# Yubo-Shankui/Bind-Your-Avatar-Implementation

Hardware: AMD Instinct MI355X
Metric: denoise-steps/sec (higher is better)
Workload: dtype bf16; 1 GPU; BASELINE.json configs[1]: full transformer.forward, 49x480x720 (13x30x45 latent tokens + 226 text), 2 characters (2 ID + 2 audio), batch 1, random-init 8.6B-param architecture; layers=42, batch=1, launch=eager, parallelism=single GPU

## Files before the change

bind_your_avatar_implementation_amd/csrc/attn_w4.hip:

```cpp
#ifndef BYA_ATTN_W4_BODY
#include "attn_common.h"
#include "gemm_persistent.h"
#include <stdlib.h>
#include "options.h"

namespace {

template <char C> struct IntTagC { static constexpr char value = C; };

constexpr int QB = 4;
constexpr int ROWS_PER_WG = 4 * QB * 32;
constexpr int RB = 128, TILE_BYTES = KV_TILE * RB, STAGE_BYTES = 2 * TILE_BYTES, NST = 3;

struct SkItem { int bh, qt, tb, nt, nt_all, role, local, slot; };

constexpr int SK_SLOT_FLOATS = 4 * QB * 2 * 16 * 64 + 4 * QB * 64;
constexpr int SK_FLAG_BYTES = 4096;

#define BYA_ATTN_W4_BODY
template <bool SK>
__global__ __launch_bounds__(256, 1) void attn_joint_w4_kernel(AttnArgs p) {
    constexpr int MXF = -1;
    const AttnMxOut* const mx = nullptr;
#include __FILE__
// ... 234 lines not shown
            MASKPAD(sacc[1][1], 32);
            { float t1_0; float t1_1; float t1_2; float t1_3; float t1_4; float t1_5; float t1_6; float t1_7; float t1_8; float t1_9; float t1_10; float t1_11; float t1_12; float t1_13; float t1_14; float t1_15; uint32_t w2_0; uint32_t w2_1; uint32_t w2_2; uint32_t w2_3; uint32_t w3_0; uint32_t w3_1; uint32_t w3_2; uint32_t w3_3; asm volatile("v_mfma_f32_32x32x16_bf16 %0, %28, %29, 0\n\tv_exp_f32 %1, %30\n\tv_exp_f32 %2, %31\n\tv_mfma_f32_32x32x16_bf16 %0, %32, %33, %0\n\tv_exp_f32 %3, %34\n\tv_add_f32 %5, %5, %1\n\tv_exp_f32 %4, %35\n\tv_add_f32 %6, %6, %2\n\tv_cvt_pk_bf16_f32 %7, %1, %2\n\tv_mfma_f32_32x32x16_bf16 %0, %36, %37, %0\n\tv_exp_f32 %8, %38\n\tv_add_f32 %5, %5, %3\n\tv_exp_f32 %9, %39\n\tv_add_f32 %6, %6, %4\n\tv_cvt_pk_bf16_f32 %10, %3, %4\n\tv_mfma_f32_32x32x16_bf16 %0, %40, %41, %0\n\tv_exp_f32 %11, %42\n\tv_add_f32 %5, %5, %8\n\tv_exp_f32 %12, %43\n\tv_add_f32 %6, %6, %9\n\tv_cvt_pk_bf16_f32 %13, %8, %9\n\tv_mfma_f32_32x32x16_bf16 %14, %44, %29, 0\n\tv_exp_f32 %15, %45\n\tv_add_f32 %5, %5, %11\n\tv_exp_f32 %16, %46\n\tv_add_f32 %6, %6, %12\n\tv_cvt_pk_bf16_f32 %17, %11, %12\n\tv_mfma_f32_32x32x16_bf16 %14, %47, %33, %14\n\tv_exp_f32 %18, %48\n\tv_add_f32 %5, %5, %15\n\tv_exp_f32 %19, %49\n\tv_add_f32 %6, %6, %16\n\tv_cvt_pk_bf16_f32 %20, %15, %16\n\tv_mfma_f32_32x32x16_bf16 %14, %50, %37, %14\n\tv_exp_f32 %21, %51\n\tv_add_f32 %5, %5, %18\n\tv_exp_f32 %22, %52\n\tv_add_f32 %6, %6, %19\n\tv_cvt_pk_bf16_f32 %23, %18, %19\n\tv_mfma_f32_32x32x16_bf16 %14, %53, %41, %14\n\tv_exp_f32 %24, %54\n\tv_add_f32 %5, %5, %21\n\tv_exp_f32 %25, %55\n\tv_add_f32 %6, %6, %22\n\tv_cvt_pk_bf16_f32 %26, %21, %22\n\tv_add_f32 %5, %5, %24\n\tv_add_f32 %6, %6, %25\n\tv_cvt_pk_bf16_f32 %27, %24, %25" : "=&v"(sacc[0][0]), "=&v"(t1_0), "=&v"(t1_1), "=&v"(t1_2), "=&v"(t1_3), "+v"(psum[1][0]), "+v"(psum[1][1]), "=&v"(w2_0), "=&v"(t1_4), "=&v"(t1_5), "=&v"(w2_1), "=&v"(t1_6), "=&v"(t1_7), "=&v"(w2_2), "=&v"(sacc[0][1]), "=&v"(t1_8), "=&v"(t1_9), "=&v"(w2_3), "=&v"(t1_10), "=&v"(t1_11), "=&v"(w3_0), "=&v"(t1_12), "=&v"(t1_13), "=&v"(w3_1), "=&v"(t1_14), "=&v"(t1_15), "=&v"(w3_2), "=&v"(w3_3) : "v"(kf[0][0]), "a"(qf[2][0]), "v"(sacc[1][1][0]), "v"(sacc[1][1][1]), "v"(kf[0][1]), "a"(qf[2][1]), "v"(sacc[1][1][2]), "v"(sacc[1][1][3]), "v"(kf[0][2]), "a"(qf[2][2]), "v"(sacc[1][1][4]), "v"(sacc[1][1][5]), "v"(kf[0][3]), "a"(qf[2][3]), "v"(sacc[1][1][6]), "v"(sacc[1][1][7]), "v"(kf[1][0]), "v"(sacc[1][1][8]), "v"(sacc[1][1][9]), "v"(kf[1][1]), "v"(sacc[1][1][10]), "v"(sacc[1][1][11]), "v"(kf[1][2]), "v"(sacc[1][1][12]), "v"(sacc[1][1][13]), "v"(kf[1][3]), "v"(sacc[1][1][14]), "v"(sacc[1][1][15]) : "memory"); pf[1][2][0] = w2_0; pf[1][2][1] = w2_1; pf[1][2][2] = w2_2; pf[1][2][3] = w2_3; pf[1][3][0] = w3_0; pf[1][3][1] = w3_1; pf[1][3][2] = w3_2; pf[1][3][3] = w3_3; }
            MASKPAD(sacc[0][0], 0);
            { const u32x4 vv0_0 = {vh[0][0][0][0], vh[0][0][0][1], vh[0][0][1][0], vh[0][0][1][1]}; const u32x4 vv1_0 = {vh[1][0][0][0], vh[1][0][0][1], vh[1][0][1][0], vh[1][0][1][1]}; const u32x4 vv0_1 = {vh[0][1][0][0], vh[0][1][0][1], vh[0][1][1][0], vh[0][1][1][1]}; const u32x4 vv1_1 = {vh[1][1][0][0], vh[1][1][0][1], vh[1][1][1][0], vh[1][1][1][1]}; const u32x4 vv0_2 = {vh[0][2][0][0], vh[0][2][0][1], vh[0][2][1][0], vh[0][2][1][1]}; const u32x4 vv1_2 = {vh[1][2][0][0], vh[1][2][0][1], vh[1][2][1][0], vh[1][2][1][1]}; const u32x4 vv0_3 = {vh[0][3][0][0], vh[0][3][0][1], vh[0][3][1][0], vh[0][3][1][1]}; const u32x4 vv1_3 = {vh[1][3][0][0], vh[1][3][0][1], vh[1][3][1][0], vh[1][3][1][1]}; float t0_0; float t0_1; float t0_2; float t0_3; float t0_4; float t0_5; float t0_6; float t0_7; float t0_8; float t0_9; float t0_10; float t0_11; float t0_12; float t0_13; float t0_14; float t0_15; uint32_t w0_0; uint32_t w0_1; uint32_t w0_2; uint32_t w0_3; uint32_t w1_0; uint32_t w1_1; uint32_t w1_2; uint32_t w1_3; asm volatile("v_mfma_f32_32x32x16_bf16 %0, %28, %29, %0\n\tv_exp_f32 %1, %30\n\tv_exp_f32 %2, %31\n\tv_mfma_f32_32x32x16_bf16 %3, %32, %29, %3\n\tv_exp_f32 %4, %33\n\tv_add_f32 %6, %6, %1\n\tv_exp_f32 %5, %34\n\tv_add_f32 %7, %7, %2\n\tv_cvt_pk_bf16_f32 %8, %1, %2\n\tv_mfma_f32_32x32x16_bf16 %0, %35, %36, %0\n\tv_exp_f32 %9, %37\n\tv_add_f32 %6, %6, %4\n\tv_exp_f32 %10, %38\n\tv_add_f32 %7, %7, %5\n\tv_cvt_pk_bf16_f32 %11, %4, %5\n\tv_mfma_f32_32x32x16_bf16 %3, %39, %36, %3\n\tv_exp_f32 %12, %40\n\tv_add_f32 %6, %6, %9\n\tv_exp_f32 %13, %41\n\tv_add_f32 %7, %7, %10\n\tv_cvt_pk_bf16_f32 %14, %9, %10\n\tv_mfma_f32_32x32x16_bf16 %0, %42, %43, %0\n\tv_exp_f32 %15, %44\n\tv_add_f32 %6, %6, %12\n\tv_exp_f32 %16, %45\n\tv_add_f32 %7, %7, %13\n\tv_cvt_pk_bf16_f32 %17, %12, %13\n\tv_mfma_f32_32x32x16_bf16 %3, %46, %43, %3\n\tv_exp_f32 %18, %47\n\tv_add_f32 %6, %6, %15\n\tv_exp_f32 %19, %48\n\tv_add_f32 %7, %7, %16\n\tv_cvt_pk_bf16_f32 %20, %15, %16\n\tv_mfma_f32_32x32x16_bf16 %0, %49, %50, %0\n\tv_exp_f32 %21, %51\n\tv_add_f32 %6, %6, %18\n\tv_exp_f32 %22, %52\n\tv_add_f32 %7, %7, %19\n\tv_cvt_pk_bf16_f32 %23, %18, %19\n\tv_mfma_f32_32x32x16_bf16 %3, %53, %50, %3\n\tv_exp_f32 %24, %54\n\tv_add_f32 %6, %6, %21\n\tv_exp_f32 %25, %55\n\tv_add_f32 %7, %7, %22\n\tv_cvt_pk_bf16_f32 %26, %21, %22\n\tv_add_f32 %6, %6, %24\n\tv_add_f32 %7, %7, %25\n\tv_cvt_pk_bf16_f32 %27, %24, %25" : "+a"(oacc[1][0]), "=&v"(t0_0), "=&v"(t0_1), "+a"(oacc[1][1]), "=&v"(t0_2), "=&v"(t0_3), "+v"(psum[2][0]), "+v"(psum[2][1]), "=&v"(w0_0), "=&v"(t0_4), "=&v"(t0_5), "=&v"(w0_1), "=&v"(t0_6), "=&v"(t0_7), "=&v"(w0_2), "=&v"(t0_8), "=&v"(t0_9), "=&v"(w0_3), "=&v"(t0_10), "=&v"(t0_11), "=&v"(w1_0), "=&v"(t0_12), "=&v"(t0_13), "=&v"(w1_1), "=&v"(t0_14), "=&v"(t0_15), "=&v"(w1_2), "=&v"(w1_3) : "v"(vv0_0), "v"(pf[1][0]), "v"(sacc[0][0][0]), "v"(sacc[0][0][1]), "v"(vv1_0), "v"(sacc[0][0][2]), "v"(sacc[0][0][3]), "v"(vv0_1), "v"(pf[1][1]), "v"(sacc[0][0][4]), "v"(sacc[0][0][5]), "v"(vv1_1), "v"(sacc[0][0][6]), "v"(sacc[0][0][7]), "v"(vv0_2), "v"(pf[1][2]), "v"(sacc[0][0][8]), "v"(sacc[0][0][9]), "v"(vv1_2), "v"(sacc[0][0][10]), "v"(sacc[0][0][11]), "v"(vv0_3), "v"(pf[1][3]), "v"(sacc[0][0][12]), "v"(sacc[0][0][13]), "v"(vv1_3), "v"(sacc[0][0][14]), "v"(sacc[0][0][15]) : "memory"); pf[0][0][0] = w0_0; pf[0][0][1] = w0_1; pf[0][0][2] = w0_2; pf[0][0][3] = w0_3; pf[0][1][0] = w1_0; pf[0][1][1] = w1_1; pf[0][1][2] = w1_2; pf[0][1][3] = w1_3; }
            MASKPAD(sacc[0][1], 32);
            { float t1_0; float t1_1; float t1_2; float t1_3; float t1_4; float t1_5; float t1_6; float t1_7; float t1_8; float t1_9; float t1_10; float t1_11; float t1_12; float t1_13; float t1_14; float t1_15; uint32_t w2_0; uint32_t w2_1; uint32_t w2_2; uint32_t w2_3; uint32_t w3_0; uint32_t w3_1; uint32_t w3_2; uint32_t w3_3; asm volatile("v_mfma_f32_32x32x16_bf16 %0, %28, %29, 0\n\tv_exp_f32 %1, %30\n\tv_exp_f32 %2, %31\n\tv_mfma_f32_32x32x16_bf16 %0, %32, %33, %0\n\tv_exp_f32 %3, %34\n\tv_add_f32 %5, %5, %1\n\tv_exp_f32 %4, %35\n\tv_add_f32 %6, %6, %2\n\tv_cvt_pk_bf16_f32 %7, %1, %2\n\tv_mfma_f32_32x32x16_bf16 %0, %36, %37, %0\n\tv_exp_f32 %8, %38\n\tv_add_f32 %5, %5, %3\n\tv_exp_f32 %9, %39\n\tv_add_f32 %6, %6, %4\n\tv_cvt_pk_bf16_f32 %10, %3, %4\n\tv_mfma_f32_32x32x16_bf16 %0, %40, %41, %0\n\tv_exp_f32 %11, %42\n\tv_add_f32 %5, %5, %8\n\tv_exp_f32 %12, %43\n\tv_add_f32 %6, %6, %9\n\tv_cvt_pk_bf16_f32 %13, %8, %9\n\tv_mfma_f32_32x32x16_bf16 %14, %44, %29, 0\n\tv_exp_f32 %15, %45\n\tv_add_f32 %5, %5, %11\n\tv_exp_f32 %16, %46\n\tv_add_f32 %6, %6, %12\n\tv_cvt_pk_bf16_f32 %17, %11, %12\n\tv_mfma_f32_32x32x16_bf16 %14, %47, %33, %14\n\tv_exp_f32 %18, %48\n\tv_add_f32 %5, %5, %15\n\tv_exp_f32 %19, %49\n\tv_add_f32 %6, %6, %16\n\tv_cvt_pk_bf16_f32 %20, %15, %16\n\tv_mfma_f32_32x32x16_bf16 %14, %50, %37, %14\n\tv_exp_f32 %21, %51\n\tv_add_f32 %5, %5, %18\n\tv_exp_f32 %22, %52\n\tv_add_f32 %6, %6, %19\n\tv_cvt_pk_bf16_f32 %23, %18, %19\n\tv_mfma_f32_32x32x16_bf16 %14, %53, %41, %14\n\tv_exp_f32 %24, %54\n\tv_add_f32 %5, %5, %21\n\tv_exp_f32 %25, %55\n\tv_add_f32 %6, %6, %22\n\tv_cvt_pk_bf16_f32 %26, %21, %22\n\tv_add_f32 %5, %5, %24\n\tv_add_f32 %6, %6, %25\n\tv_cvt_pk_bf16_f32 %27, %24, %25" : "=&v"(sacc[1][0]), "=&v"(t1_0), "=&v"(t1_1), "=&v"(t1_2), "=&v"(t1_3), "+v"(psum[2][0]), "+v"(psum[2][1]), "=&v"(w2_0), "=&v"(t1_4), "=&v"(t1_5), "=&v"(w2_1), "=&v"(t1_6), "=&v"(t1_7), "=&v"(w2_2), "=&v"(sacc[1][1]), "=&v"(t1_8), "=&v"(t1_9), "=&v"(w2_3), "=&v"(t1_10), "=&v"(t1_11), "=&v"(w3_0), "=&v"(t1_12), "=&v"(t1_13), "=&v"(w3_1), "=&v"(t1_14), "=&v"(t1_15), "=&v"(w3_2), "=&v"(w3_3) : "v"(kf[0][0]), "a"(qf[3][0]), "v"(sacc[0][1][0]), "v"(sacc[0][1][1]), "v"(kf[0][1]), "a"(qf[3][1]), "v"(sacc[0][1][2]), "v"(sacc[0][1][3]), "v"(kf[0][2]), "a"(qf[3][2]), "v"(sacc[0][1][4]), "v"(sacc[0][1][5]), "v"(kf[0][3]), "a"(qf[3][3]), "v"(sacc[0][1][6]), "v"(sacc[0][1][7]), "v"(kf[1][0]), "v"(sacc[0][1][8]), "v"(sacc[0][1][9]), "v"(kf[1][1]), "v"(sacc[0][1][10]), "v"(sacc[0][1][11]), "v"(kf[1][2]), "v"(sacc[0][1][12]), "v"(sacc[0][1][13]), "v"(kf[1][3]), "v"(sacc[0][1][14]), "v"(sacc[0][1][15]) : "memory"); pf[0][2][0] = w2_0; pf[0][2][1] = w2_1; pf[0][2][2] = w2_2; pf[0][2][3] = w2_3; pf[0][3][0] = w3_0; pf[0][3][1] = w3_1; pf[0][3][2] = w3_2; pf[0][3][3] = w3_3; }
            MASKPAD(sacc[1][0], 0);
            { const u32x4 vv0_0 = {vh[0][0][0][0], vh[0][0][0][1], vh[0][0][1][0], vh[0][0][1][1]}; const u32x4 vv1_0 = {vh[1][0][0][0], vh[1][0][0][1], vh[1][0][1][0], vh[1][0][1][1]}; const u32x4 vv0_1 = {vh[0][1][0][0], vh[0][1][0][1], vh[0][1][1][0], vh[0][1][1][1]}; const u32x4 vv1_1 = {vh[1][1][0][0], vh[1][1][0][1], vh[1][1][1][0], vh[1][1][1][1]}; const u32x4 vv0_2 = {vh[0][2][0][0], vh[0][2][0][1], vh[0][2][1][0], vh[0][2][1][1]}; const u32x4 vv1_2 = {vh[1][2][0][0], vh[1][2][0][1], vh[1][2][1][0], vh[1][2][1][1]}; const u32x4 vv0_3 = {vh[0][3][0][0], vh[0][3][0][1], vh[0][3][1][0], vh[0][3][1][1]}; const u32x4 vv1_3 = {vh[1][3][0][0], vh[1][3][0][1], vh[1][3][1][0], vh[1][3][1][1]}; const uint32_t dma_dst0 = dma_dst + 0 + 0 * TILE_BYTES; const uint32_t dma_dst1 = dma_dst + 1024 + 0 * TILE_BYTES; const uint32_t dma_dst2 = dma_dst + 0 + 1 * TILE_BYTES; const uint32_t dma_dst3 = dma_dst + 1024 + 1 * TILE_BYTES; float t0_0; float t0_1; float t0_2; float t0_3; float t0_4; float t0_5; float t0_6; float t0_7; float t0_8; float t0_9; float t0_10; float t0_11; float t0_12; float t0_13; float t0_14; float t0_15; uint32_t w0_0; uint32_t w0_1; uint32_t w0_2; uint32_t w0_3; uint32_t w1_0; uint32_t w1_1; uint32_t w1_2; uint32_t w1_3; asm volatile("v_mfma_f32_32x32x16_bf16 %0, %36, %37, %0\n\ts_waitcnt vmcnt(4)\n\ts_barrier\n\tds_read_b128 %1, %38 offset:0\n\tds_read_b128 %2, %39 offset:0\n\tv_exp_f32 %3, %40\n\tv_exp_f32 %4, %41\n\tv_mfma_f32_32x32x16_bf16 %5, %42, %37, %5\n\tds_read_b128 %6, %43 offset:0\n\tds_read_b128 %7, %44 offset:0\n\tv_exp_f32 %8, %45\n\tv_add_f32 %10, %10, %3\n\tv_exp_f32 %9, %46\n\tv_add_f32 %11, %11, %4\n\tv_cvt_pk_bf16_f32 %12, %3, %4\n\tv_mfma_f32_32x32x16_bf16 %0, %47, %48, %0\n\tds_read_b128 %13, %38 offset:4096\n\tds_read_b128 %14, %39 offset:4096\n\tv_exp_f32 %15, %49\n\tv_add_f32 %10, %10, %8\n\tv_exp_f32 %16, %50\n\tv_add_f32 %11, %11, %9\n\tv_cvt_pk_bf16_f32 %17, %8, %9\n\tv_mfma_f32_32x32x16_bf16 %5, %51, %48, %5\n\tds_read_b128 %18, %43 offset:4096\n\tds_read_b128 %19, %44 offset:4096\n\tv_exp_f32 %20, %52\n\tv_add_f32 %10, %10, %15\n\tv_exp_f32 %21, %53\n\tv_add_f32 %11, %11, %16\n\tv_cvt_pk_bf16_f32 %22, %15, %16\n\tv_mfma_f32_32x32x16_bf16 %0, %54, %55, %0\n\ts_mov_b32 m0, %56\n\ts_nop 0\n\tbuffer_load_dwordx4 %57, %58, %59 offen lds\n\tv_exp_f32 %23, %60\n\tv_add_f32 %10, %10, %20\n\tv_exp_f32 %24, %61\n\tv_add_f32 %11, %11, %21\n\tv_cvt_pk_bf16_f32 %25, %20, %21\n\tv_mfma_f32_32x32x16_bf16 %5, %62, %55, %5\n\ts_mov_b32 m0, %63\n\ts_nop 0\n\tbuffer_load_dwordx4 %64, %58, %59 offen lds\n\tv_exp_f32 %26, %65\n\tv_add_f32 %10, %10, %23\n\tv_exp_f32 %27, %66\n\tv_add_f32 %11, %11, %24\n\tv_cvt_pk_bf16_f32 %28, %23, %24\n\tv_mfma_f32_32x32x16_bf16 %0, %67, %68, %0\n\ts_mov_b32 m0, %69\n\ts_nop 0\n\tbuffer_load_dwordx4 %70, %71, %72 offen lds\n\tv_exp_f32 %29, %73\n\tv_add_f32 %10, %10, %26\n\tv_exp_f32 %30, %74\n\tv_add_f32 %11, %11, %27\n\tv_cvt_pk_bf16_f32 %31, %26, %27\n\tv_mfma_f32_32x32x16_bf16 %5, %75, %68, %5\n\ts_mov_b32 m0, %76\n\ts_nop 0\n\tbuffer_load_dwordx4 %77, %71, %72 offen lds\n\tv_exp_f32 %32, %78\n\tv_add_f32 %10, %10, %29\n\tv_exp_f32 %33, %79\n\tv_add_f32 %11, %11, %30\n\tv_cvt_pk_bf16_f32 %34, %29, %30\n\tv_add_f32 %10, %10, %32\n\tv_add_f32 %11, %11, %33\n\tv_cvt_pk_bf16_f32 %35, %32, %33\n\ts_waitcnt lgkmcnt(0)" : "+a"(oacc[2][0]), "=&v"(kf[0][0]), "=&v"(kf[0][1]), "=&v"(t0_0), "=&v"(t0_1), "+a"(oacc[2][1]), "=&v"(kf[0][2]), "=&v"(kf[0][3]), "=&v"(t0_2), "=&v"(t0_3), "+v"(psum[3][0]), "+v"(psum[3][1]), "=&v"(w0_0), "=&v"(kf[1][0]), "=&v"(kf[1][1]), "=&v"(t0_4), "=&v"(t0_5), "=&v"(w0_1), "=&v"(kf[1][2]), "=&v"(kf[1][3]), "=&v"(t0_6), "=&v"(t0_7), "=&v"(w0_2), "=&v"(t0_8), "=&v"(t0_9), "=&v"(w0_3), "=&v"(t0_10), "=&v"(t0_11), "=&v"(w1_0), "=&v"(t0_12), "=&v"(t0_13), "=&v"(w1_1), "=&v"(t0_14), "=&v"(t0_15), "=&v"(w1_2), "=&v"(w1_3) : "v"(vv0_0), "v"(pf[0][0]), "v"(kaddr[0]), "v"(kaddr[1]), "v"(sacc[1][0][0]), "v"(sacc[1][0][1]), "v"(vv1_0), "v"(kaddr[2]), "v"(kaddr[3]), "v"(sacc[1][0][2]), "v"(sacc[1][0][3]), "v"(vv0_1), "v"(pf[0][1]), "v"(sacc[1][0][4]), "v"(sacc[1][0][5]), "v"(vv1_1), "v"(sacc[1][0][6]), "v"(sacc[1][0][7]), "v"(vv0_2), "v"(pf[0][2]), "s"(dma_dst0), "v"(dvo[0]), "s"(rsK), "s"(soffK), "v"(sacc[1][0][8]), "v"(sacc[1][0][9]), "v"(vv1_2), "s"(dma_dst1), "v"(dvo[1]), "v"(sacc[1][0][10]), "v"(sacc[1][0][11]), "v"(vv0_3), "v"(pf[0][3]), "s"(dma_dst2), "v"(dvo[2]), "s"(rsV), "s"(soffV), "v"(sacc[1][0][12]), "v"(sacc[1][0][13]), "v"(vv1_3), "s"(dma_dst3), "v"(dvo[3]), "v"(sacc[1][0][14]), "v"(sacc[1][0][15]) : "memory"); pf[1][0][0] = w0_0; pf[1][0][1] = w0_1; pf[1][0][2] = w0_2; pf[1][0][3] = w0_3; pf[1][1][0] = w1_0; pf[1][1][1] = w1_1; pf[1][1][2] = w1_2; pf[1][1][3] = w1_3; }
            MASKPAD(sacc[1][1], 32);
        } else if constexpr (VAR == 'T') {
            { float t1_0; float t1_1; float t1_2; float t1_3; float t1_4; float t1_5; float t1_6; float t1_7; float t1_8; float t1_9; float t1_10; float t1_11; float t1_12; float t1_13; float t1_14; float t1_15; uint32_t w2_0; uint32_t w2_1; uint32_t w2_2; uint32_t w2_3; uint32_t w3_0; uint32_t w3_1; uint32_t w3_2; uint32_t w3_3; asm volatile("v_exp_f32 %0, %26\n\tv_exp_f32 %1, %27\n\tv_exp_f32 %2, %28\n\tv_add_f32 %4, %4, %0\n\tv_exp_f32 %3, %29\n\tv_add_f32 %5, %5, %1\n\tv_cvt_pk_bf16_f32 %6, %0, %1\n\tv_exp_f32 %7, %30\n\tv_add_f32 %4, %4, %2\n\tv_exp_f32 %8, %31\n\tv_add_f32 %5, %5, %3\n\tv_cvt_pk_bf16_f32 %9, %2, %3\n\tv_exp_f32 %10, %32\n\tv_add_f32 %4, %4, %7\n\tv_exp_f32 %11, %33\n\tv_add_f32 %5, %5, %8\n\tv_cvt_pk_bf16_f32 %12, %7, %8\n\tv_exp_f32 %13, %34\n\tv_add_f32 %4, %4, %10\n\tv_exp_f32 %14, %35\n\tv_add_f32 %5, %5, %11\n\tv_cvt_pk_bf16_f32 %15, %10, %11\n\tv_exp_f32 %16, %36\n\tv_add_f32 %4, %4, %13\n\tv_exp_f32 %17, %37\n\tv_add_f32 %5, %5, %14\n\tv_cvt_pk_bf16_f32 %18, %13, %14\n\tv_exp_f32 %19, %38\n\tv_add_f32 %4, %4, %16\n\tv_exp_f32 %20, %39\n\tv_add_f32 %5, %5, %17\n\tv_cvt_pk_bf16_f32 %21, %16, %17\n\tv_exp_f32 %22, %40\n\tv_add_f32 %4, %4, %19\n\tv_exp_f32 %23, %41\n\tv_add_f32 %5, %5, %20\n\tv_cvt_pk_bf16_f32 %24, %19, %20\n\tv_add_f32 %4, %4, %22\n\tv_add_f32 %5, %5, %23\n\tv_cvt_pk_bf16_f32 %25, %22, %23" : "=&v"(t1_0), "=&v"(t1_1), "=&v"(t1_2), "=&v"(t1_3), "+v"(psum[3][0]), "+v"(psum[3][1]), "=&v"(w2_0), "=&v"(t1_4), "=&v"(t1_5), "=&v"(w2_1), "=&v"(t1_6), "=&v"(t1_7), "=&v"(w2_2), "=&v"(t1_8), "=&v"(t1_9), "=&v"(w2_3), "=&v"(t1_10), "=&v"(t1_11), "=&v"(w3_0), "=&v"(t1_12), "=&v"(t1_13), "=&v"(w3_1), "=&v"(t1_14), "=&v"(t1_15), "=&v"(w3_2), "=&v"(w3_3) : "v"(sacc[1][1][0]), "v"(sacc[1][1][1]), "v"(sacc[1][1][2]), "v"(sacc[1][1][3]), "v"(sacc[1][1][4]), "v"(sacc[1][1][5]), "v"(sacc[1][1][6]), "v"(sacc[1][1][7]), "v"(sacc[1][1][8]), "v"(sacc[1][1][9]), "v"(sacc[1][1][10]), "v"(sacc[1][1][11]), "v"(sacc[1][1][12]), "v"(sacc[1][1][13]), "v"(sacc[1][1][14]), "v"(sacc[1][1][15]) : "memory"); pf[1][2][0] = w2_0; pf[1][2][1] = w2_1; pf[1][2][2] = w2_2; pf[1][2][3] = w2_3; pf[1][3][0] = w3_0; pf[1][3][1] = w3_1; pf[1][3][2] = w3_2; pf[1][3][3] = w3_3; }
            { const u32x4 vv0_0 = {vh[0][0][0][0], vh[0][0][0][1], vh[0][0][1][0], vh[0][0][1][1]}; const u32x4 vv1_0 = {vh[1][0][0][0], vh[1][0][0][1], vh[1][0][1][0], vh[1][0][1][1]}; const u32x4 vv0_1 = {vh[0][1][0][0], vh[0][1][0][1], vh[0][1][1][0], vh[0][1][1][1]}; const u32x4 vv1_1 = {vh[1][1][0][0], vh[1][1][0][1], vh[1][1][1][0], vh[1][1][1][1]}; const u32x4 vv0_2 = {vh[0][2][0][0], vh[0][2][0][1], vh[0][2][1][0], vh[0][2][1][1]}; const u32x4 vv1_2 = {vh[1][2][0][0], vh[1][2][0][1], vh[1][2][1][0], vh[1][2][1][1]}; const u32x4 vv0_3 = {vh[0][3][0][0], vh[0][3][0][1], vh[0][3][1][0], vh[0][3][1][1]}; const u32x4 vv1_3 = {vh[1][3][0][0], vh[1][3][0][1], vh[1][3][1][0], vh[1][3][1][1]}; asm volatile("v_mfma_f32_32x32x16_bf16 %0, %2, %3, %0\n\tv_mfma_f32_32x32x16_bf16 %1, %4, %3, %1\n\tv_mfma_f32_32x32x16_bf16 %0, %5, %6, %0\n\tv_mfma_f32_32x32x16_bf16 %1, %7, %6, %1\n\tv_mfma_f32_32x32x16_bf16 %0, %8, %9, %0\n\tv_mfma_f32_32x32x16_bf16 %1, %10, %9, %1\n\tv_mfma_f32_32x32x16_bf16 %0, %11, %12, %0\n\tv_mfma_f32_32x32x16_bf16 %1, %13, %12, %1" : "+a"(oacc[3][0]), "+a"(oacc[3][1]) : "v"(vv0_0), "v"(pf[1][0]), "v"(vv1_0), "v"(vv0_1), "v"(pf[1][1]), "v"(vv1_1), "v"(vv0_2), "v"(pf[1][2]), "v"(vv1_2), "v"(vv0_3), "v"(pf[1][3]), "v"(vv1_3) : "memory"); }
        }
    };

    bool first_item = true;
    for (;;) {
        if (SK) {
            int item;
            if (sk_round < sk_rfull) {
                item = sk_round * sk_ncu + sk_idx;
                ++sk_round;
                it.tb = 0; it.nt = nt_all; it.role = 0; it.local = 0;
            } else if (sk_idx < sk_rem) {
                if (sk_main_done) break;
                sk_main_done = true;
                it.local = sk_idx;
                item = sk_rfull * sk_ncu + it.local;
                it.tb = 0; it.nt = sk_a; it.role = sk_suf ? 2 : 0; it.slot = 0;
            } else {
                if (sk_s >= sk_end) break;
                it.local = sk_s / sk_suf;
                item = sk_rfull * sk_ncu + it.local;
                const int off = sk_s - it.local * sk_suf, left = sk_end - sk_s;
                it.tb = sk_a + off;
                it.nt = sk_suf - off < left ? sk_suf - off : left;
                it.role = 1;
                it.slot = sk_xcd * (2 * sk_ncu) + (sk_idx - sk_rem) + it.local;
                sk_s += it.nt;
            }
            it.nt_all = nt_all;
            if (nbh % 8 == 0) {
                it.bh = (item / p.nqt) * 8 + sk_xcd;
                it.qt = item % p.nqt;
            } else {
                it.bh = (sk_base + item) / p.nqt;
                it.qt = (sk_base + item) % p.nqt;
            }
            if (!first_item) asm volatile("s_barrier" ::: "memory");
            first_item = false;
        }
        if (p.bound_dev) {
            const float* tq = p.bound_dev + (long long)lane * 2 * p.bound_heads + p.bound_bh0 + it.bh;
            float q2 = lane < p.bound_slots ? tq[0] : 0.f, k2 = lane < p.bound_slots ? tq[p.bound_heads] : 0.f;
#pragma unroll
            for (int o = 32; o > 0; o >>= 1) {
                q2 = fmaxf(q2, __shfl_xor(q2, o, 64));
                k2 = fmaxf(k2, __shfl_xor(k2, o, 64));
            }
            const bool skip = !(sqrtf(q2) * sqrtf(k2) <= p.bound_limit);
            if (tid == 0) p.fallback[it.bh] = skip ? 1 : 0;
            if (skip) {
                if (SK) continue;
                return;
            }
        }
        const int head = it.bh % p.heads, b12 = it.bh / p.heads;
        const int b1 = b12 / p.nb2, b2 = b12 % p.nb2;
        const bf16_t* Qp = p.q + b1 * p.q_s1 + b2 * p.q_s2 + (long long)head * D;
        const bf16_t* Kp = p.k + b1 * p.k_s1 + b2 * p.k_s2 + (long long)head * D + (long long)it.tb * KV_TILE * p.k_row;
        const bf16_t* Vp = p.v + b1 * p.v_s1 + b2 * p.v_s2 + (long long)head * D + (long long)it.tb * KV_TILE * p.v_row;
        bf16_t* Op = p.o + b1 * p.o_s1 + b2 * p.o_s2 + (long long)head * D;
        uint8_t* Cp = nullptr;
        uint8_t* Sp = nullptr;
        if constexpr (MXF >= 0) {
            Cp = reinterpret_cast<uint8_t*>(p.o) + b1 * p.o_s1 + b2 * p.o_s2 + (long long)head * 2 * mx_block_bytes(MXF);
            Sp = mx->scales + b1 * mx->s1 + b2 * mx->s2 + 2 * head;
        }
        const int skv_left = p.Skv - it.tb * KV_TILE;
        rsK = raw_rsrc(Kp, (uint32_t)(((long long)(skv_left - 1) * p.k_row + D) * 2));
        rsV = raw_rsrc(Vp, (uint32_t)(((long long)(skv_left - 1) * p.v_row + D) * 2));
        const int ntiles = it.nt;
        stage_tile(0, 0);
        stage_tile(1, 1);
        stage_tile(2, 2);

        const int q0 = it.qt * ROWS_PER_WG + wave * (QB * 32);
#pragma unroll
        for (int b = 0; b < QB; ++b) {
            int qrow = q0 + b * 32 + r;
            q_valid[b] = qrow < p.Sq;
            qrow = q_valid[b] ? qrow : p.Sq - 1;
#pragma unroll
            for (int s = 0; s < 4; ++s)
                qf[b][s] = __builtin_bit_cast(bf16x8, *reinterpret_cast<const u32x4*>(Qp + (long long)qrow * p.q_row + s * 16 + hf * 8));
        }
#pragma unroll
        for (int b = 0; b < QB; ++b) {
            psum[b][0] = psum[b][1] = 0.f;
#pragma unroll
            for (int d = 0; d < 2; ++d)
#pragma unroll
                for (int i = 0; i < 16; ++i) oacc[b][d][i] = 0.f;
        }
#pragma unroll
        for (int i = 0; i < 16; ++i) { sacc[0][0][i] = 0.f; sacc[0][1][i] = 0.f; sacc[1][0][i] = 0.f; sacc[1][1][i] = -INFINITY; }
#pragma unroll
        for (int x = 0; x < 2; ++x)
#pragma unroll
            for (int ks = 0; ks < 4; ++ks) {
                pf[x][ks] = u32x4{0u, 0u, 0u, 0u};
                vh[x][ks][0] = u32x2{0u, 0u};
                vh[x][ks][1] = u32x2{0u, 0u};
            }

#pragma unroll
        for (int b = 0; b < QB; ++b)
#pragma unroll
            for (int s = 0; s < 4; ++s) asm volatile("" : "+a"(qf[b][s]));
        VMC(8);
        BAR();
        {
            uint32_t kaddr[4];
#pragma unroll
            for (int s = 0; s < 4; ++s) kaddr[s] = kofs[s];
            RK(0, 0); RK(0, 1); RK(0, 2); RK(0, 3); RK(1, 0); RK(1, 1); RK(1, 2); RK(1, 3);
            LGKM(0);
        }
        int st = 0;
        for (int t = 0; t < ntiles - 1; ++t) {
            const int st1 = st == NST - 1 ? 0 : st + 1;
            uint32_t kaddr[4], vaddr[2];
#pragma unroll
            for (int s = 0; s < 4; ++s) kaddr[s] = kofs[s] + st1 * STAGE_BYTES;
#pragma unroll
            for (int d = 0; d < 2; ++d) vaddr[d] = vofs[d] + st * STAGE_BYTES;
            body(IntTagC<'L'>{}, kaddr, vaddr, lds0s + st * STAGE_BYTES, (uint32_t)(t + 3) * k_tile_stride,
                 (uint32_t)(t + 3) * v_tile_stride);
            st = st1;
        }
        {
            const int t = ntiles - 1, st1 = st == NST - 1 ? 0 : st + 1;
            keys_last = skv_left - t * KV_TILE;
            uint32_t kaddr[4], vaddr[2];
#pragma unroll
            for (int s = 0; s < 4; ++s) kaddr[s] = kofs[s] + st1 * STAGE_BYTES;
#pragma unroll
            for (int d = 0; d < 2; ++d) vaddr[d] = vofs[d] + st * STAGE_BYTES;
            body(IntTagC<'M'>{}, kaddr, vaddr, lds0s + st * STAGE_BYTES, (uint32_t)(t + 3) * k_tile_stride,
                 (uint32_t)(t + 3) * v_tile_stride);
        }
        {
            const uint32_t none4[4] = {0u, 0u, 0u, 0u}, none2[2] = {0u, 0u};
            body(IntTagC<'T'>{}, none4, none2, 0u, 0u, 0u);
        }
        asm volatile("s_nop 15\n\ts_nop 15\n\ts_waitcnt vmcnt(0)" ::: "memory");

        if (SK && it.role == 1) {
            const int my_slot = it.slot;
            float* const slot = p.sk_part + (size_t)my_slot * SK_SLOT_FLOATS;
#pragma unroll
            for (int b = 0; b < QB; ++b) {
#pragma unroll
                for (int d = 0; d < 2; ++d)
#pragma unroll
                    for (int gq = 0; gq < 4; ++gq) {
                        f32x4 w = {oacc[b][d][gq * 4 + 0], oacc[b][d][gq * 4 + 1], oacc[b][d][gq * 4 + 2], oacc[b][d][gq * 4 + 3]};
                        *reinterpret_cast<f32x4*>(slot + ((size_t)(((wave * QB + b) * 2 + d) * 4 + gq) * 64 + lane) * 4) = w;
                    }
                slot[4 * QB * 2 * 16 * 64 + (wave * QB + b) * 64 + lane] = psum[b][0] + psum[b][1];
            }
            __builtin_amdgcn_fence(__ATOMIC_RELEASE, "agent");
// ... 27 lines not shown
#pragma unroll
                    for (int d = 0; d < 2; ++d)
#pragma unroll
                        for (int gq = 0; gq < 4; ++gq) {
                            const f32x4 w = *reinterpret_cast<const f32x4*>(slot + ((size_t)(((wave * QB + b) * 2 + d) * 4 + gq) * 64 + lane) * 4);
                            oacc[b][d][gq * 4 + 0] += w[0]; oacc[b][d][gq * 4 + 1] += w[1];
                            oacc[b][d][gq * 4 + 2] += w[2]; oacc[b][d][gq * 4 + 3] += w[3];
                        }
                    psum[b][0] += slot[4 * QB * 2 * 16 * 64 + (wave * QB + b) * 64 + lane];
                    asm volatile("s_waitcnt vmcnt(0)" ::: "memory");
                }
                asm volatile("s_waitcnt vmcnt(0)" ::: "memory");
                asm volatile("s_barrier" ::: "memory");
                if (tid == 0) __hip_atomic_store(p.sk_flags + cs, 0u, __ATOMIC_RELAXED, __HIP_MEMORY_SCOPE_AGENT);
            }
        }

#pragma unroll
        for (int b = 0; b < QB; ++b) {
            const float l_half = psum[b][0] + psum[b][1];
            const auto lsw = __builtin_amdgcn_permlane32_swap(__float_as_uint(l_half), __float_as_uint(l_half), false, false);
            const float inv = 1.0f / (__uint_as_float(lsw[0]) + __uint_as_float(lsw[1]));
            if constexpr (MXF >= 0) {
                const long long row = q_valid[b] ? q0 + b * 32 + r : 0;
                store_mx_head<MXF>(Cp + row * p.o_row, Sp + row * mx->row, oacc[b][0], oacc[b][1], inv, hf, q_valid[b]);
            } else {
            bf16_t* orow = Op + (long long)(q_valid[b] ? q0 + b * 32 + r : 0) * p.o_row;
#pragma unroll
            for (int d = 0; d < 2; ++d) store_o_tile(orow + d * 32, oacc[b][d], inv, hf, q_valid[b], p.o_wide != 0);
            }
        }
        if (!SK) break;
    }
#endif
```

Before: 2.873 steps/s.

## Carry K/V and Q prefetch across stream-K work items in attention kernel

In the persistent stream-K attention kernel, each work item now looks up the next item ahead of time. It switches the K/V buffer resources partway through the current item's tile loop, so the last few pipeline stages already prefetch the next item's first K/V tiles into LDS. It also issues the next item's Q loads before the tail and epilogue. This hides the per-item pipeline fill and Q load latency between consecutive items, at the cost of much more complex stage and offset bookkeeping. Role-1 (partial) items now run the epilogue and break afterward.

After: 2.871 steps/s (median of 2 runs). About the same (-0.1%).

```diff
diff --git a/bind_your_avatar_implementation_amd/csrc/attn_w4.hip b/bind_your_avatar_implementation_amd/csrc/attn_w4.hip
--- a/bind_your_avatar_implementation_amd/csrc/attn_w4.hip
+++ b/bind_your_avatar_implementation_amd/csrc/attn_w4.hip
@@ -272,62 +272,106 @@
         }
     };
 
-    bool first_item = true;
-    for (;;) {
-        if (SK) {
+    auto head_over_bound = [&](int bh) -> bool {
+        const float* tq = p.bound_dev + (long long)lane * 2 * p.bound_heads + p.bound_bh0 + bh;
+        float q2 = lane < p.bound_slots ? tq[0] : 0.f, k2 = lane < p.bound_slots ? tq[p.bound_heads] : 0.f;
+#pragma unroll
+        for (int o = 32; o > 0; o >>= 1) {
+            q2 = fmaxf(q2, __shfl_xor(q2, o, 64));
+            k2 = fmaxf(k2, __shfl_xor(k2, o, 64));
+        }
+        const bool skip = !(sqrtf(q2) * sqrtf(k2) <= p.bound_limit);
+        if (tid == 0) p.fallback[bh] = skip ? 1 : 0;
+        return __builtin_amdgcn_readfirstlane(skip ? 1 : 0) != 0;
+    };
+    auto walk = [&](SkItem& n) -> bool {
+        for (;;) {
             int item;
             if (sk_round < sk_rfull) {
                 item = sk_round * sk_ncu + sk_idx;
                 ++sk_round;
-                it.tb = 0; it.nt = nt_all; it.role = 0; it.local = 0;
+                n.tb = 0; n.nt = nt_all; n.role = 0; n.local = 0; n.slot = 0;
             } else if (sk_idx < sk_rem) {
-                if (sk_main_done) break;
+                if (sk_main_done) return false;
                 sk_main_done = true;
-                it.local = sk_idx;
-                item = sk_rfull * sk_ncu + it.local;
-                it.tb = 0; it.nt = sk_a; it.role = sk_suf ? 2 : 0; it.slot = 0;
+                n.local = sk_idx;
+                item = sk_rfull * sk_ncu + n.local;
+                n.tb = 0; n.nt = sk_a; n.role = sk_suf ? 2 : 0; n.slot = 0;
             } else {
-                if (sk_s >= sk_end) break;
-                it.local = sk_s / sk_suf;
-                item = sk_rfull * sk_ncu + it.local;
-                const int off = sk_s - it.local * sk_suf, left = sk_end - sk_s;
-                it.tb = sk_a + off;
-                it.nt = sk_suf - off < left ? sk_suf - off : left;
-                it.role = 1;
-                it.slot = sk_xcd * (2 * sk_ncu) + (sk_idx - sk_rem) + it.local;
-                sk_s += it.nt;
-            }
-            it.nt_all = nt_all;
+                if (sk_s >= sk_end) return false;
+                n.local = sk_s / sk_suf;
+                item = sk_rfull * sk_ncu + n.local;
+                const int off = sk_s - n.local * sk_suf, left = sk_end - sk_s;
+                n.tb = sk_a + off;
+                n.nt = sk_suf - off < left ? sk_suf - off : left;
+                n.role = 1;
+                n.slot = sk_xcd * (2 * sk_ncu) + (sk_idx - sk_rem) + n.local;
+                sk_s += n.nt;
+            }
+            n.nt_all = nt_all;
             if (nbh % 8 == 0) {
-                it.bh = (item / p.nqt) * 8 + sk_xcd;
-                it.qt = item % p.nqt;
+                n.bh = (item / p.nqt) * 8 + sk_xcd;
+                n.qt = item % p.nqt;
             } else {
-                it.bh = (sk_base + item) / p.nqt;
-                it.qt = (sk_base + item) % p.nqt;
-            }
-            if (!first_item) asm volatile("s_barrier" ::: "memory");
+                n.bh = (sk_base + item) / p.nqt;
+                n.qt = (sk_base + item) % p.nqt;
+            }
+            if (!p.bound_dev || !head_over_bound(n.bh)) return true;
+        }
+    };
+    auto item_kv = [&](const SkItem& n, i32x4& rk, i32x4& rv) {
+        const int head = n.bh % p.heads, b12 = n.bh / p.heads;
+        const int b1 = b12 / p.nb2, b2 = b12 % p.nb2;
+        const bf16_t* Kp = p.k + b1 * p.k_s1 + b2 * p.k_s2 + (long long)head * D + (long long)n.tb * KV_TILE * p.k_row;
+        const bf16_t* Vp = p.v + b1 * p.v_s1 + b2 * p.v_s2 + (long long)head * D + (long long)n.tb * KV_TILE * p.v_row;
+        const int left = p.Skv - n.tb * KV_TILE;
+        rk = raw_rsrc(Kp, (uint32_t)(((long long)(left - 1) * p.k_row + D) * 2));
+        rv = raw_rsrc(Vp, (uint32_t)(((long long)(left - 1) * p.v_row + D) * 2));
+    };
+    auto request_q = [&](const SkItem& n) {
+        const int head = n.bh % p.heads, b12 = n.bh / p.heads;
+        const int b1 = b12 / p.nb2, b2 = b12 % p.nb2;
+        const bf16_t* Qn = p.q + b1 * p.q_s1 + b2 * p.q_s2 + (long long)head * D + hf * 8;
+        const int qn0 = n.qt * ROWS_PER_WG + wave * (QB * 32);
+#pragma unroll
+        for (int b = 0; b < QB; ++b) {
+            int qrow = qn0 + b * 32 + r;
+            qrow = qrow < p.Sq ? qrow : p.Sq - 1;
+            const bf16_t* src = Qn + (long long)qrow * p.q_row;
+#define QL(S) asm volatile("global_load_dwordx4 %0, %1, off offset:%2" : "=a"(qf[b][S]) : "v"(src), "i"((S) * 32) : "memory")
+            QL(0); QL(1); QL(2); QL(3);
+#undef QL
+        }
+    };
+#ifdef BYA_ATTN_W4_NO_CARRY
+    constexpr bool CARRY = false;
+#else
+    constexpr bool CARRY = SK;
+#endif
+
+    SkItem nx;
+    i32x4 rsKn, rsVn;
+    if (SK && !walk(it)) return;
+    bool first_item = true, has_next = false, fed = false;
+    int st = 0;
+    int carried = 0;
+    for (;;) {
+        if (SK) {
+            if (!first_item) {
+                if (!has_next) break;
+                carried = fed ? (it.nt < NST ? it.nt : NST) : 0;
+                it = nx;
+                asm volatile("s_barrier" ::: "memory");
+            }
             first_item = false;
-        }
-        if (p.bound_dev) {
-            const float* tq = p.bound_dev + (long long)lane * 2 * p.bound_heads + p.bound_bh0 + it.bh;
-            float q2 = lane < p.bound_slots ? tq[0] : 0.f, k2 = lane < p.bound_slots ? tq[p.bound_heads] : 0.f;
-#pragma unroll
-            for (int o = 32; o > 0; o >>= 1) {
-                q2 = fmaxf(q2, __shfl_xor(q2, o, 64));
-                k2 = fmaxf(k2, __shfl_xor(k2, o, 64));
-            }
-            const bool skip = !(sqrtf(q2) * sqrtf(k2) <= p.bound_limit);
-            if (tid == 0) p.fallback[it.bh] = skip ? 1 : 0;
-            if (skip) {
-                if (SK) continue;
-                return;
-            }
-        }
+            has_next = walk(nx);
+            fed = CARRY && has_next;
+            if (fed) item_kv(nx, rsKn, rsVn);
+        }
+        if (!SK && p.bound_dev && head_over_bound(it.bh)) return;
         const int head = it.bh % p.heads, b12 = it.bh / p.heads;
         const int b1 = b12 / p.nb2, b2 = b12 % p.nb2;
         const bf16_t* Qp = p.q + b1 * p.q_s1 + b2 * p.q_s2 + (long long)head * D;
-        const bf16_t* Kp = p.k + b1 * p.k_s1 + b2 * p.k_s2 + (long long)head * D + (long long)it.tb * KV_TILE * p.k_row;
-        const bf16_t* Vp = p.v + b1 * p.v_s1 + b2 * p.v_s2 + (long long)head * D + (long long)it.tb * KV_TILE * p.v_row;
         bf16_t* Op = p.o + b1 * p.o_s1 + b2 * p.o_s2 + (long long)head * D;
         uint8_t* Cp = nullptr;
         uint8_t* Sp = nullptr;
@@ -336,66 +380,87 @@
             Sp = mx->scales + b1 * mx->s1 + b2 * mx->s2 + 2 * head;
         }
         const int skv_left = p.Skv - it.tb * KV_TILE;
-        rsK = raw_rsrc(Kp, (uint32_t)(((long long)(skv_left - 1) * p.k_row + D) * 2));
-        rsV = raw_rsrc(Vp, (uint32_t)(((long long)(skv_left - 1) * p.v_row + D) * 2));
+        item_kv(it, rsK, rsV);
         const int ntiles = it.nt;
-        stage_tile(0, 0);
-        stage_tile(1, 1);
-        stage_tile(2, 2);
-
         const int q0 = it.qt * ROWS_PER_WG + wave * (QB * 32);
-#pragma unroll
-        for (int b = 0; b < QB; ++b) {
-            int qrow = q0 + b * 32 + r;
-            q_valid[b] = qrow < p.Sq;
-            qrow = q_valid[b] ? qrow : p.Sq - 1;
-#pragma unroll
-            for (int s = 0; s < 4; ++s)
-                qf[b][s] = __builtin_bit_cast(bf16x8, *reinterpret_cast<const u32x4*>(Qp + (long long)qrow * p.q_row + s * 16 + hf * 8));
-        }
-#pragma unroll
-        for (int b = 0; b < QB; ++b) {
-            psum[b][0] = psum[b][1] = 0.f;
-#pragma unroll
-            for (int d = 0; d < 2; ++d)
-#pragma unroll
-                for (int i = 0; i < 16; ++i) oacc[b][d][i] = 0.f;
-        }
-#pragma unroll
-        for (int i = 0; i < 16; ++i) { sacc[0][0][i] = 0.f; sacc[0][1][i] = 0.f; sacc[1][0][i] = 0.f; sacc[1][1][i] = -INFINITY; }
-#pragma unroll
-        for (int x = 0; x < 2; ++x)
-#pragma unroll
-            for (int ks = 0; ks < 4; ++ks) {
-                pf[x][ks] = u32x4{0u, 0u, 0u, 0u};
-                vh[x][ks][0] = u32x2{0u, 0u};
-                vh[x][ks][1] = u32x2{0u, 0u};
-            }
-
-#pragma unroll
-        for (int b = 0; b < QB; ++b)
-#pragma unroll
-            for (int s = 0; s < 4; ++s) asm volatile("" : "+a"(qf[b][s]));
-        VMC(8);
-        BAR();
+        auto zero_state = [&]() {
+#pragma unroll
+            for (int b = 0; b < QB; ++b) {
+                psum[b][0] = psum[b][1] = 0.f;
+#pragma unroll
+                for (int d = 0; d < 2; ++d)
+#pragma unroll
+                    for (int i = 0; i < 16; ++i) oacc[b][d][i] = 0.f;
+            }
+#pragma unroll
+            for (int i = 0; i < 16; ++i) { sacc[0][0][i] = 0.f; sacc[0][1][i] = 0.f; sacc[1][0][i] = 0.f; sacc[1][1][i] = -INFINITY; }
+#pragma unroll
+            for (int x = 0; x < 2; ++x)
+#pragma unroll
+                for (int ks = 0; ks < 4; ++ks) {
+                    pf[x][ks] = u32x4{0u, 0u, 0u, 0u};
+                    vh[x][ks][0] = u32x2{0u, 0u};
+                    vh[x][ks][1] = u32x2{0u, 0u};
+                }
+        };
+        if (carried == 0) {
+            st = 0;
+            stage_tile(0, 0);
+            stage_tile(1, 1);
+            stage_tile(2, 2);
+#pragma unroll
+            for (int b = 0; b < QB; ++b) {
+                int qrow = q0 + b * 32 + r;
+                q_valid[b] = qrow < p.Sq;
+                qrow = q_valid[b] ? qrow : p.Sq - 1;
+#pragma unroll
+                for (int s = 0; s < 4; ++s)
+                    qf[b][s] = __builtin_bit_cast(bf16x8, *reinterpret_cast<const u32x4*>(Qp + (long long)qrow * p.q_row + s * 16 + hf * 8));
+            }
+            zero_state();
+#pragma unroll
+            for (int b = 0; b < QB; ++b)
+#pragma unroll
+                for (int s = 0; s < 4; ++s) asm volatile("" : "+a"(qf[b][s]));
+            VMC(8);
+            BAR();
+        } else {
+            if (carried < NST) {
+                stage_tile(0, st);
+                if (carried == 1) stage_tile(1, st == NST - 1 ? 0 : st + 1);
+                VMC(0);
+                BAR();
+            }
+#pragma unroll
+            for (int b = 0; b < QB; ++b) q_valid[b] = q0 + b * 32 + r < p.Sq;
+            zero_state();
+        }
         {
             uint32_t kaddr[4];
 #pragma unroll
-            for (int s = 0; s < 4; ++s) kaddr[s] = kofs[s];
+            for (int s = 0; s < 4; ++s) kaddr[s] = kofs[s] + st * STAGE_BYTES;
             RK(0, 0); RK(0, 1); RK(0, 2); RK(0, 3); RK(1, 0); RK(1, 1); RK(1, 2); RK(1, 3);
             LGKM(0);
         }
-        int st = 0;
-        for (int t = 0; t < ntiles - 1; ++t) {
+        auto tile = [&](int t, int toff) {
             const int st1 = st == NST - 1 ? 0 : st + 1;
             uint32_t kaddr[4], vaddr[2];
 #pragma unroll
             for (int s = 0; s < 4; ++s) kaddr[s] = kofs[s] + st1 * STAGE_BYTES;
 #pragma unroll
             for (int d = 0; d < 2; ++d) vaddr[d] = vofs[d] + st * STAGE_BYTES;
-            body(IntTagC<'L'>{}, kaddr, vaddr, lds0s + st * STAGE_BYTES, (uint32_t)(t + 3) * k_tile_stride,
-                 (uint32_t)(t + 3) * v_tile_stride);
+            body(IntTagC<'L'>{}, kaddr, vaddr, lds0s + st * STAGE_BYTES, (uint32_t)(t + toff) * k_tile_stride,
+                 (uint32_t)(t + toff) * v_tile_stride);
             st = st1;
+        };
+        int toff = 3;
+        const int t_fed = !fed ? ntiles - 1 : ntiles > 3 ? ntiles - 3 : 0;
+        for (int t = 0; t < t_fed; ++t) tile(t, 3);
+        if (fed) {
+            rsK = rsKn;
+            rsV = rsVn;
+            toff = 3 - ntiles;
+            for (int t = t_fed; t < ntiles - 1; ++t) tile(t, toff);
         }
         {
             const int t = ntiles - 1, st1 = st == NST - 1 ? 0 : st + 1;
@@ -405,15 +470,39 @@
             for (int s = 0; s < 4; ++s) kaddr[s] = kofs[s] + st1 * STAGE_BYTES;
 #pragma unroll
             for (int d = 0; d < 2; ++d) vaddr[d] = vofs[d] + st * STAGE_BYTES;
-            body(IntTagC<'M'>{}, kaddr, vaddr, lds0s + st * STAGE_BYTES, (uint32_t)(t + 3) * k_tile_stride,
-                 (uint32_t)(t + 3) * v_tile_stride);
-        }
+            body(IntTagC<'M'>{}, kaddr, vaddr, lds0s + st * STAGE_BYTES, (uint32_t)(t + toff) * k_tile_stride,
+                 (uint32_t)(t + toff) * v_tile_stride);
+            st = st1;
+        }
+        if (fed) request_q(nx);
         {
             const uint32_t none4[4] = {0u, 0u, 0u, 0u}, none2[2] = {0u, 0u};
             body(IntTagC<'T'>{}, none4, none2, 0u, 0u, 0u);
         }
         asm volatile("s_nop 15\n\ts_nop 15\n\ts_waitcnt vmcnt(0)" ::: "memory");
-
+        if (fed) {
+#pragma unroll
+            for (int b = 0; b < QB; ++b)
+#pragma unroll
+                for (int s = 0; s < 4; ++s) asm volatile("" : "+a"(qf[b][s]));
+        }
+
+        auto epilogue = [&]() {
+#pragma unroll
+        for (int b = 0; b < QB; ++b) {
+            const float l_half = psum[b][0] + psum[b][1];
+            const auto lsw = __builtin_amdgcn_permlane32_swap(__float_as_uint(l_half), __float_as_uint(l_half), false, false);
+            const float inv = 1.0f / (__uint_as_float(lsw[0]) + __uint_as_float(lsw[1]));
+            if constexpr (MXF >= 0) {
+                const long long row = q_valid[b] ? q0 + b * 32 + r : 0;
+                store_mx_head<MXF>(Cp + row * p.o_row, Sp + row * mx->row, oacc[b][0], oacc[b][1], inv, hf, q_valid[b]);
+            } else {
+            bf16_t* orow = Op + (long long)(q_valid[b] ? q0 + b * 32 + r : 0) * p.o_row;
+#pragma unroll
+            for (int d = 0; d < 2; ++d) store_o_tile(orow + d * 32, oacc[b][d], inv, hf, q_valid[b], p.o_wide != 0);
+            }
+        }
+        };
         if (SK && it.role == 1) {
             const int my_slot = it.slot;
             float* const slot = p.sk_part + (size_t)my_slot * SK_SLOT_FLOATS;
@@ -471,22 +560,11 @@
                 asm volatile("s_barrier" ::: "memory");
                 if (tid == 0) __hip_atomic_store(p.sk_flags + cs, 0u, __ATOMIC_RELAXED, __HIP_MEMORY_SCOPE_AGENT);
             }
-        }
-
-#pragma unroll
-        for (int b = 0; b < QB; ++b) {
-            const float l_half = psum[b][0] + psum[b][1];
-            const auto lsw = __builtin_amdgcn_permlane32_swap(__float_as_uint(l_half), __float_as_uint(l_half), false, false);
-            const float inv = 1.0f / (__uint_as_float(lsw[0]) + __uint_as_float(lsw[1]));
-            if constexpr (MXF >= 0) {
-                const long long row = q_valid[b] ? q0 + b * 32 + r : 0;
-                store_mx_head<MXF>(Cp + row * p.o_row, Sp + row * mx->row, oacc[b][0], oacc[b][1], inv, hf, q_valid[b]);
-            } else {
-            bf16_t* orow = Op + (long long)(q_valid[b] ? q0 + b * 32 + r : 0) * p.o_row;
-#pragma unroll
-            for (int d = 0; d < 2; ++d) store_o_tile(orow + d * 32, oacc[b][d], inv, hf, q_valid[b], p.o_wide != 0);
-            }
-        }
+            epilogue();
+            break;
+        }
+
+        epilogue();
         if (!SK) break;
     }
 #endif
```
